# m4tx/idencomp

Measured on NVIDIA B200. Metric: fastq_compress_decompress_GBps, higher is better.
Workload: dtype u32

## Files before the change

### idencomp_b200/csrc/idn_gpu.cu

```cuda
#include "../../include/idn_gpu.h"

#include <algorithm>
#include <cstdarg>
#include <cstdio>
#include <chrono>
#include <cstring>
#include <string>
#include <vector>

#include "idn_fastq.cuh"
#include "idn_native.cuh"

using namespace idn;

namespace {

struct DevBuf {
    void* p = nullptr;
    size_t cap = 0;
    cudaError_t ensure(size_t n) {
        if (n <= cap) return cudaSuccess;
        if (p) cudaFree(p);
        p = nullptr;
        cap = 0;
// ... 248 lines not shown
#endif
    for (int i = 0; i < kNumStaticPairs; i++) {
        bool same = true;
        for (int k = 0; k < 5; k++)
            same = same && ctx->slots[acid_slot].spec_tuple[k] == kStaticPairs[i][k] && ctx->slots[q_slot].spec_tuple[k] == kStaticPairs[i][5 + k];
        if (same) return i;
    }
    return -1;
}

extern "C" int32_t idn_gpu_kernel_variant(const idn_gpu_ctx* ctx, idn_model_t acid_model, idn_model_t q_model) {
    if (!ctx) return -1;
    for (idn_model_t h : {acid_model, q_model})
        if (h < 0 || (size_t)h >= ctx->slots.size() || !ctx->slots[h].used) return -1;
    if (ctx->slots[acid_model].dev.type != IDN_MODEL_ACID || ctx->slots[q_model].dev.type != IDN_MODEL_QSCORE) return -1;
    return static_pair_index(ctx, acid_model, q_model);
}
extern "C" int32_t idn_gpu_kernel_variant_count(void) { return kNumStaticPairs; }

static unsigned debug_smem() {
    static const unsigned v = [] { const char* e = getenv("IDN_DEBUG_SMEM"); return e ? (unsigned)atoi(e) : 0u; }();
    return v;
}
#define IDN_LAUNCH_UNIFORM(idx, KERNEL, grid, st, ...)                                         \
    switch (idx) {                                                                             \
        case 0: KERNEL<true, SP0><<<grid, 128, debug_smem(), st>>>(__VA_ARGS__); break;                   \
        case 1: KERNEL<true, SP1><<<grid, 128, debug_smem(), st>>>(__VA_ARGS__); break;                   \
        case 2: KERNEL<true, SP2><<<grid, 128, debug_smem(), st>>>(__VA_ARGS__); break;                   \
        case 3: KERNEL<true, SP3><<<grid, 128, debug_smem(), st>>>(__VA_ARGS__); break;                   \
        case 4: KERNEL<true, SP4><<<grid, 128, debug_smem(), st>>>(__VA_ARGS__); break;                   \
        case 5: KERNEL<true, SP5><<<grid, 128, debug_smem(), st>>>(__VA_ARGS__); break;                   \
        case 6: KERNEL<true, SP6><<<grid, 128, debug_smem(), st>>>(__VA_ARGS__); break;                   \
        case 7: KERNEL<true, SP7><<<grid, 128, debug_smem(), st>>>(__VA_ARGS__); break;                   \
        default: KERNEL<true, DynSpecs><<<grid, 128, debug_smem(), st>>>(__VA_ARGS__); break;             \
    }

#define IDN_LAUNCH_LIST(idx, KERNEL, grid, st, ...)                                            \
    switch (idx) {                                                                             \
        case 0: KERNEL<SP0><<<grid, 128, debug_smem(), st>>>(__VA_ARGS__); break;                         \
        case 1: KERNEL<SP1><<<grid, 128, debug_smem(), st>>>(__VA_ARGS__); break;                         \
        case 2: KERNEL<SP2><<<grid, 128, debug_smem(), st>>>(__VA_ARGS__); break;                         \
        case 3: KERNEL<SP3><<<grid, 128, debug_smem(), st>>>(__VA_ARGS__); break;                         \
        case 4: KERNEL<SP4><<<grid, 128, debug_smem(), st>>>(__VA_ARGS__); break;                         \
        case 5: KERNEL<SP5><<<grid, 128, debug_smem(), st>>>(__VA_ARGS__); break;                         \
        case 6: KERNEL<SP6><<<grid, 128, debug_smem(), st>>>(__VA_ARGS__); break;                         \
        case 7: KERNEL<SP7><<<grid, 128, debug_smem(), st>>>(__VA_ARGS__); break;                         \
        default: KERNEL<DynSpecs><<<grid, 128, debug_smem(), st>>>(__VA_ARGS__); break;                   \
    }

extern "C" int32_t idn_gpu_abi_version(void) { return IDN_GPU_ABI_VERSION; }

extern "C" int32_t idn_gpu_device_count(void) {
    int n = 0;
    if (cudaGetDeviceCount(&n) != cudaSuccess) {
        (void)cudaGetLastError();
        return 0;
    }
    return n;
}

static void make_crc_tables(uint32_t* tab, uint32_t* xpow) {
    for (uint32_t i = 0; i < 256; i++) {
        uint32_t c = i;
        for (int k = 0; k < 8; k++) c = (c >> 1) ^ ((c & 1) ? 0xEDB88320u : 0);
        tab[i] = c;
    }
    auto mul = [](uint32_t a, uint32_t b) {
        uint32_t p = 0;
        for (int i = 0; i < 32; i++) {
            if (b & 0x80000000u) p ^= a;
            a = (a >> 1) ^ ((a & 1) ? 0xEDB88320u : 0);
            b <<= 1;
        }
        return p;
    };
    xpow[0] = 0x00800000u;
    for (int k = 1; k < 64; k++) xpow[k] = mul(xpow[k - 1], xpow[k - 1]);
}

static void make_crc_back_tables(const uint32_t* tab, const uint32_t* xpow, uint32_t* back ) {
    uint32_t rtop[256];
    for (uint32_t i = 0; i < 256; i++) rtop[tab[i] >> 24] = i;
    uint32_t* tinv = back;
    uint32_t* u = back + 256;
    for (uint32_t t = 0; t < 256; t++) tinv[t] = (tab[rtop[t]] << 8) | rtop[t];
    auto linv = [&](uint32_t v) { return (v << 8) ^ tinv[v >> 24]; };
    for (uint32_t b = 0; b < 256; b++) u[b] = linv(tab[b]);
    auto mul = [](uint32_t a, uint32_t b) {
        uint32_t p = 0;
        for (int i = 0; i < 32; i++) {
            if (b & 0x80000000u) p ^= a;
            a = (a >> 1) ^ ((a & 1) ? 0xEDB88320u : 0);
            b <<= 1;
        }
        return p;
    };
    uint32_t* xlen = back + 512;
    uint32_t x = 0x80000000u;
    for (uint32_t n = 0; n < kCrcLenTab; n++) {
        xlen[2 * n] = x;
        xlen[2 * n + 1] = mul(x, x);
        x = mul(x, xpow[0]);
    }
}

extern "C" int32_t idn_gpu_create(int32_t device, idn_gpu_ctx** out) {
    if (!out) return IDN_E_INVALID_ARG;
    *out = nullptr;
    int n = idn_gpu_device_count();
    if (n <= 0 || device < 0 || device >= n) return IDN_E_CUDA;
    idn_gpu_ctx* ctx = new idn_gpu_ctx();
    ctx->device = device;
    if (const char* pb = getenv("IDN_PIPE_BLOCKS")) {
        ctx->pipe_blocks = std::max(1, atoi(pb));
        ctx->pipe_blocks_set = true;
    }
    if (getenv("IDN_NO_BUCKETS")) ctx->bucket_pairs = false;
    if (const char* w = getenv("IDN_WALK")) ctx->walk_mode = strcmp(w, "serial") == 0 ? 1 : (strcmp(w, "fast") == 0 ? 2 : 0);
    auto bail = [&](const char* what) {
        fprintf(stderr, "idn_gpu_create: %s failed: %s\n", what, cudaGetErrorString(cudaGetLastError()));
        delete ctx;
        return (int32_t)IDN_E_CUDA;
    };
    if (cudaSetDevice(device) != cudaSuccess) return bail("cudaSetDevice");
    if (cudaDeviceGetAttribute(&ctx->sm_count, cudaDevAttrMultiProcessorCount, device) != cudaSuccess) return bail("cudaDeviceGetAttribute");
    if (cudaStreamCreateWithFlags(&ctx->stream, cudaStreamNonBlocking) != cudaSuccess) return bail("cudaStreamCreate");
    if (cudaEventCreateWithFlags(&ctx->ev, cudaEventDisableTiming | cudaEventBlockingSync) != cudaSuccess) return bail("cudaEventCreate");
    if (cudaMalloc(&ctx->d_models, sizeof(ModelDev) * kMaxSlots) != cudaSuccess) return bail("cudaMalloc");
    if (cudaMemset(ctx->d_models, 0, sizeof(ModelDev) * kMaxSlots) != cudaSuccess) return bail("cudaMemset");
    uint32_t tab[256], xpow[64];
    make_crc_tables(tab, xpow);
    if (cudaMalloc(&ctx->d_crc_tab, sizeof tab) != cudaSuccess) return bail("cudaMalloc");
    if (cudaMalloc(&ctx->d_xpow, sizeof xpow) != cudaSuccess) return bail("cudaMalloc");
    if (cudaMemcpy(ctx->d_crc_tab, tab, sizeof tab, cudaMemcpyHostToDevice) != cudaSuccess) return bail("cudaMemcpy");
    if (cudaMemcpy(ctx->d_xpow, xpow, sizeof xpow, cudaMemcpyHostToDevice) != cudaSuccess) return bail("cudaMemcpy");
    {
        std::vector<uint32_t> back(512 + 2 * kCrcLenTab);
        make_crc_back_tables(tab, xpow, back.data());
        if (cudaMalloc(&ctx->d_crc_back, back.size() * 4) != cudaSuccess) return bail("cudaMalloc");
        if (cudaMemcpy(ctx->d_crc_back, back.data(), back.size() * 4, cudaMemcpyHostToDevice) != cudaSuccess) return bail("cudaMemcpy");
    }
    if (getenv("IDN_NO_ENC_CRC")) ctx->enc_crc = false;
    *out = ctx;
    return IDN_OK;
}

static void pipe_destroy(idn_gpu_pipe* p);

extern "C" void idn_gpu_destroy(idn_gpu_ctx* ctx) {
    if (!ctx) return;
    cudaSetDevice(ctx->device);
    cudaDeviceSynchronize();
    for (auto& s : ctx->slots)
        if (s.used) s.free_all();
    DevBuf* bufs[] = {&ctx->w_scratch, &ctx->w_paylen,  &ctx->w_sizes,   &ctx->w_chosen,     &ctx->w_tiles,  &ctx->w_sliceoff,
                      &ctx->w_readblock, &ctx->w_small, &ctx->w_crcpart, &ctx->w_crclen,     &ctx->w_index,  &ctx->w_blk,
                      &ctx->w_lanefirst, &ctx->w_laneoff, &ctx->w_laneblock, &ctx->w_blkinfo, &ctx->w_nhdr, &ctx->w_lanesym, &ctx->w_walkdone, &ctx->w_blockadj,
                      &ctx->f_text, &ctx->f_tilecnt, &ctx->f_tilebase, &ctx->f_linestart, &ctx->f_linefn, &ctx->f_linestate, &ctx->f_tilefn,
                      &ctx->f_tilestate, &ctx->f_recscan, &ctx->f_title, &ctx->f_namelo, &ctx->f_namelen, &ctx->f_readlen, &ctx->f_readoff,
                      &ctx->f_nameoff, &ctx->f_names, &ctx->f_acids, &ctx->f_quals, &ctx->f_err, &ctx->f_fmtoff, &ctx->f_fmttext,
                      &ctx->f_blockfirst, &ctx->f_nxt, &ctx->w_bucket, &ctx->w_list,
                      &ctx->s_acids,   &ctx->s_quals,   &ctx->s_readoff, &ctx->s_blockfirst, &ctx->s_prefix, &ctx->s_names,
                      &ctx->s_nameoff, &ctx->s_out,     &ctx->s_blockoff, &ctx->s_crc,       &ctx->s_stats,  &ctx->s_sizes,
                      &ctx->s_blocks,  &ctx->s_blocklen, &ctx->s_aout,    &ctx->s_qout,    &ctx->s_offout,     &ctx->s_status, &ctx->s_idx};
    for (DevBuf* b : bufs) b->release();
    pipe_destroy(ctx->pipe);
    cudaFree(ctx->d_models);
    cudaFree(ctx->d_crc_tab);
    cudaFree(ctx->d_xpow);
    cudaFree(ctx->d_crc_back);
    if (ctx->ev) cudaEventDestroy(ctx->ev);
    if (ctx->stream) cudaStreamDestroy(ctx->stream);
    delete ctx;
}

extern "C" int32_t idn_gpu_host_alloc(uint64_t bytes, void** p) {
    if (!p) return IDN_E_INVALID_ARG;
    *p = nullptr;
    if (cudaHostAlloc(p, bytes ? bytes : 1, cudaHostAllocPortable) != cudaSuccess) {
        (void)cudaGetLastError();
        *p = nullptr;
        return IDN_E_CUDA;
    }
    return IDN_OK;
}
extern "C" void idn_gpu_host_free(void* p) {
    if (p) cudaFreeHost(p);
}

extern "C" int32_t idn_gpu_set_walk(idn_gpu_ctx* ctx, int32_t mode) {
    if (!ctx) return IDN_E_INVALID_ARG;
    if (mode < 0 || mode > 2) return fail(ctx, IDN_E_INVALID_ARG, "walk mode %d", mode);
    ctx->walk_mode = mode;
    return IDN_OK;
}

extern "C" int32_t idn_gpu_set_lane_symbols(idn_gpu_ctx* ctx, uint32_t lane_syms) {
    if (!ctx) return IDN_E_INVALID_ARG;
    if (lane_syms == 0) return fail(ctx, IDN_E_INVALID_ARG, "lane_syms must be positive");
    ctx->lane_syms = lane_syms;
    return IDN_OK;
}

extern "C" const char* idn_gpu_last_error(const idn_gpu_ctx* ctx) { return ctx ? ctx->err.c_str() : "no context"; }
extern "C" uint64_t idn_gpu_launch_count(const idn_gpu_ctx* ctx) { return ctx ? ctx->launches : 0; }

extern "C" int32_t idn_gpu_model_upload(idn_gpu_ctx* ctx, int32_t model_type, int32_t spec_kind, int32_t acid_order,
                                        int32_t q_order, int32_t pos_bits, int32_t q_max, uint32_t n_ctx,
                                        const uint16_t* cum, const uint32_t* spec_keys, const uint32_t* spec_ctx,
                                        uint64_t n_specs, idn_model_t* handle) {
    if (!ctx || !handle || !cum) return fail(ctx, IDN_E_INVALID_ARG, "NULL argument");
    if (model_type != IDN_MODEL_ACID && model_type != IDN_MODEL_QSCORE)
        return fail(ctx, IDN_E_INVALID_ARG, "bad model type %d", model_type);
    if (n_ctx > 65536) return fail(ctx, IDN_E_UNSUPPORTED, "model has %u contexts (limit 65536, check_model sequence_compressor.rs:209-219)", n_ctx);
    if (n_specs && (!spec_keys || !spec_ctx)) return fail(ctx, IDN_E_INVALID_ARG, "NULL spec table");
    CU(cudaSetDevice(ctx->device));
    const SpecBuild sb = make_spec(spec_kind, acid_order, q_order, pos_bits, q_max);
    const SpecDev spec = sb.spec;
    const uint32_t bits = sb.total_bits;
    if (!sb.ok)
// ... 1738 lines not shown
```

### idencomp_b200/csrc/idn_kernels.cuh

```cuda
#pragma once
#include "idn_device.cuh"

namespace idn {

struct BackReader {
    const uint32_t* wp;
    uint32_t word;
    int lane;
    __device__ __forceinline__ void start(const uint8_t* last) {
        const uintptr_t a = reinterpret_cast<uintptr_t>(last);
        wp = reinterpret_cast<const uint32_t*>(a & ~(uintptr_t)3);
        lane = (int)(a & 3) + 4;
        word = 0;
    }
    __device__ __forceinline__ uint32_t get() {
        if (lane >= 4) {
            word = __ldg(wp);
            lane -= 4;
        }
        const uint32_t b = (word >> (8 * lane)) & 0xffu;
        if (--lane < 0) {
            lane = 7;
            wp--;
        }
// ... 7 lines not shown
    int lane;
    __device__ __forceinline__ void start(const uint8_t* first) {
        const uintptr_t a = reinterpret_cast<uintptr_t>(first);
        wp = reinterpret_cast<const uint32_t*>(a & ~(uintptr_t)3);
        lane = (int)(a & 3) - 4;
        word = 0;
    }
    __device__ __forceinline__ uint32_t get() {
        if (lane < 0) {
            word = __ldg(wp);
            lane += 4;
        }
        const uint32_t b = (word >> (8 * lane)) & 0xffu;
        if (++lane == 4) {
            lane = -4;
            wp++;
        }
        return b;
    }
};

__device__ __forceinline__ uint4 load_chunk16(const uint8_t* __restrict__ base, unsigned long long n, const uint8_t* c) {
    if (c >= base && c + 16 <= base + n) return __ldg(reinterpret_cast<const uint4*>(c));
    uint32_t w[4] = {0, 0, 0, 0};
#pragma unroll
    for (int j = 0; j < 16; j++)
        if (c + j >= base && c + j < base + n) w[j >> 2] |= (uint32_t)__ldg(c + j) << (8 * (j & 3));
    return make_uint4(w[0], w[1], w[2], w[3]);
}

struct SymBackReader {
    const uint8_t *abase, *qbase;
    unsigned long long n;
    const uint8_t* c;
    uint32_t ca, cq;
    uint32_t a0, a1, a2, q0, q1, q2;
    uint32_t left;
    bool vec;
    __device__ __forceinline__ void load() {
        const uint4 va = load_chunk16(abase, n, c), vq = load_chunk16(qbase, n, qbase + (c - abase));
        ca = va.w; a2 = va.z; a1 = va.y; a0 = va.x;
        cq = vq.w; q2 = vq.z; q1 = vq.y; q0 = vq.x;
        c -= 16;
        left = 16;
    }
    __device__ __forceinline__ void next_word() {
        ca = a2; a2 = a1; a1 = a0;
        cq = q2; q2 = q1; q1 = q0;
    }
    __device__ __forceinline__ void start(const uint8_t* acids, const uint8_t* quals, unsigned long long n_symbols, long long off,
                                          uint32_t len) {
        abase = acids;
        qbase = quals;
        n = n_symbols;
        vec = ((reinterpret_cast<uintptr_t>(acids) ^ reinterpret_cast<uintptr_t>(quals)) & 15) == 0;
        ca = cq = a0 = a1 = a2 = q0 = q1 = q2 = 0;
        left = 0;
        const uint8_t* last = acids + off + (long long)len - 1;
        c = last;
        if (!vec || len == 0) return;
        const uint32_t k = (uint32_t)(reinterpret_cast<uintptr_t>(last) & 15);
        c = last - k;
        load();
        for (uint32_t t = 3; t > (k >> 2); t--) next_word();
        const uint32_t sh = 8 * (3 - (k & 3));
        ca <<= sh;
        cq <<= sh;
        left = k + 1;
    }
    __device__ __forceinline__ void get(uint32_t& a, uint32_t& q) {
        if (!vec) {
            a = __ldg(c);
            q = __ldg(qbase + (c - abase));
            c--;
            return;
        }
        if (left == 0) load();
        a = ca >> 24;
        q = cq >> 24;
        ca <<= 8;
        cq <<= 8;
        left--;
        if ((left & 3) == 0 && left != 0) next_word();
    }
};

struct BackWriter {
    uint32_t* wptr;
    unsigned long long acc;
    uint32_t nbits;
    __device__ __forceinline__ void init(uint8_t* end) {
        wptr = reinterpret_cast<uint32_t*>(end);
        acc = 0;
        nbits = 0;
    }
    __device__ __forceinline__ uint32_t bytes(const uint8_t* end) const {
        return (uint32_t)(reinterpret_cast<const uint32_t*>(end) - wptr) * 4u + (nbits >> 3);
    }
    __device__ __forceinline__ void push_bits(uint32_t bytes_be, uint32_t kbits) {
        acc = (acc << kbits) | bytes_be;
        nbits += kbits;
    }
    __device__ __forceinline__ void drain() {
        if (nbits >= 32) {
            nbits -= 32;
            *--wptr = (uint32_t)(acc >> nbits);
        }
    }
    __device__ __forceinline__ void push_u32_le(uint32_t x) {
        acc = (acc << 32) | x;
        nbits += 32;
        drain();
    }
    __device__ __forceinline__ void finish() {
        uint8_t* p = reinterpret_cast<uint8_t*>(wptr);
        const uint32_t n = nbits >> 3;
        for (uint32_t k = 0; k < n; k++) p[-1 - (int)k] = (uint8_t)(acc >> (8 * (n - 1 - k)));
    }
};

struct FwdWriter {
    uint8_t* wbase;
    uint32_t acc, lane, first;
    __device__ __forceinline__ void init(uint8_t* dst) {
        lane = (uint32_t)(reinterpret_cast<uintptr_t>(dst) & 3);
        first = lane;
        wbase = dst - lane;
        acc = 0;
    }
    __device__ __forceinline__ void push(uint32_t b) {
        acc |= b << (8 * lane);
        if (++lane == 4) {
            if (first == 0) {
                *reinterpret_cast<uint32_t*>(wbase) = acc;
            } else {
                for (uint32_t k = first; k < 4; k++) wbase[k] = (uint8_t)(acc >> (8 * k));
                first = 0;
            }
            wbase += 4;
            acc = 0;
            lane = 0;
        }
    }
    __device__ __forceinline__ void finish() {
        for (uint32_t k = first; k < lane; k++) wbase[k] = (uint8_t)(acc >> (8 * k));
    }
};

template <int M>
struct ModelPack {
    ModelDev m[M];
    uint32_t n;
};

template <int M, bool kDense>
__global__ void __launch_bounds__(128)
score_multi_kernel(const ModelPack<M> P, const uint8_t* __restrict__ acids, const uint8_t* __restrict__ quals,
                   const uint64_t* __restrict__ read_off, uint64_t n_reads, uint32_t n_cols, uint32_t col0,
                   uint32_t* __restrict__ sizes, uint32_t* __restrict__ err) {
    uint64_t r = (uint64_t)blockIdx.x * blockDim.x + threadIdx.x;
    if (r >= n_reads) return;
    uint64_t off = read_off[r];
    uint32_t len = (uint32_t)(read_off[r + 1] - off);
    uint32_t pbmax = 0;
#pragma unroll
    for (int k = 0; k < M; k++)
// ... 89 lines not shown
        uint32_t res[kMaxCand + 1];
        for (uint32_t s = 0; s <= n_cand; s++) res[s] = pick_model(sz, n_cand, s == n_cand ? NONE : s);
        for (uint32_t s = 0; s <= n_cand; s++) {
            uint32_t cur = out[s];
            out[s] = res[cur == NONE ? n_cand : cur];
        }
    }
    uint32_t in_state = NONE;
    for (uint32_t l = 0; l < 31; l++) {
        uint32_t my_out = out[in_state == NONE ? n_cand : in_state];
        uint32_t from_l = __shfl_sync(0xffffffffu, my_out, l);
        if (lane == l + 1) in_state = from_l;
    }
    uint32_t cur = in_state;
    for (uint64_t r = c0; r < c1; r++) {
        for (uint32_t k = 0; k < n_cand; k++) sz[k] = sizes ? sizes[r * n_models + cols[k]] : 0u;
        uint32_t best = pick_model(sz, n_cand, cur);
        ch[r] = (uint8_t)best;
        sw[r] = best != cur;
        cur = best;
    }
}

__global__ void switch_single_kernel(const uint32_t* __restrict__ block_first, uint32_t n_blocks, uint8_t* __restrict__ switched,
                                     uint64_t n_reads) {
    uint32_t b = blockIdx.x * blockDim.x + threadIdx.x;
    if (b >= n_blocks || block_first[b + 1] == block_first[b]) return;
    switched[block_first[b]] = 1;
    switched[n_reads + block_first[b]] = 1;
}

struct EncodeArgs {
    const ModelDev* models;
    const uint8_t* acids;
    const uint8_t* quals;
    uint64_t n_symbols;
    const uint64_t* read_off;
    uint64_t n_reads;
    int32_t fixed_acid, fixed_q;
    const uint8_t* chosen;
    const int32_t* cand_model;
    uint8_t* scratch;
    uint32_t* pay_len;
    uint32_t* err;
    const uint8_t* switched;
    const uint8_t* cand_index;
    const uint32_t* crc_back;
    const uint32_t* xpow;
    uint32_t* part_crc;
    unsigned long long* part_len;
};
struct ReadList {
    const uint32_t* list;
    const uint32_t* base;
    const uint32_t* count;
};
constexpr unsigned long long kSlotExtra = 24;

struct EncStream {
    uint32_t x0, x1;
    BackWriter out;
    bool bad;
    __device__ __forceinline__ void begin(uint8_t* slot_end) {
        x0 = x1 = kRansL;
        out.init(slot_end);
        bad = false;
    }
    __device__ __forceinline__ void flush_states() {
        out.push_u32_le(x0);
        out.push_u32_le(x1);
    }
    __device__ __forceinline__ void flush() {
        flush_states();
        out.finish();
    }
    __device__ __forceinline__ uint32_t total(const uint8_t* slot_end) const { return out.bytes(slot_end); }
};

constexpr uint32_t kCrcLenTab = 1024;
__device__ __forceinline__ uint32_t gf2_mul(uint32_t a, uint32_t b);
__device__ __forceinline__ uint32_t x8n_mod_p(unsigned long long n, const uint32_t* __restrict__ xpow);
struct EncCrc {
    const uint32_t* tinv;
    const uint32_t* u;
    uint32_t ba, bq;
    __device__ __forceinline__ void add(uint32_t a, uint32_t q) {
        ba = (ba << 8) ^ tinv[ba >> 24] ^ u[a];
        bq = (bq << 8) ^ tinv[bq >> 24] ^ u[q];
    }
};

template <class P>
__device__ __forceinline__ void encode_read_body(const ModelDev& ma, const ModelDev& mq, const uint8_t* __restrict__ acids,
                                                 const uint8_t* __restrict__ quals, unsigned long long n_symbols, long long off,
                                                 uint32_t len, uint32_t p0, uint32_t p1, EncStream& S, EncCrc& C) {
    constexpr SpecDev ksa = P::sa(), ksq = P::sq();
    const SpecDev& sa = P::kStatic ? ksa : ma.spec;
    const SpecDev& sq = P::kStatic ? ksq : mq.spec;
#ifndef IDN_NO_SYM16
    SymBackReader rs;
    rs.start(acids, quals, n_symbols, off, p1);
#else
    (void)n_symbols;
    BackReader ra, rq;
    ra.start(acids + off + p1 - 1);
    rq.start(quals + off + p1 - 1);
#endif
    GenBack ga, gq;
    ga.clear(sa);
    gq.clear(sq);
    int32_t front = (int32_t)p1 - 1;
    uint32_t raw_a = 0;
    unsigned long long raw_q = 0;
    auto pull = [&]() {
        uint32_t a = 0, q = 0;
        if (front >= 0) {
#ifndef IDN_NO_SYM16
            rs.get(a, q);
#else
            a = ra.get();
            q = rq.get();
#endif
            if (a > 4 || q > 93) {
                S.bad = true;
                a = a > 4 ? 0 : a;
                q = q > 93 ? 0 : q;
            }
            if (C.tinv) C.add(a, q);
        }
        front--;
        const bool z = a * q == 0;
        ga.shift_in(sa, a, q, z);
        gq.shift_in(sq, a, q, z);
        raw_a = (raw_a >> 3) | (a << (3 * kHist));
        raw_q = (raw_q >> 7) | ((unsigned long long)q << (7 * kHist));
    };
#pragma unroll 1
    for (int t = 0; t < kHist; t++) pull();
    ga.init_state(sa);
    gq.init_state(sq);
    const uint32_t pbmax = sa.pb > sq.pb ? sa.pb : sq.pb;
    const uint32_t psa = pbmax - sa.pb, psq = pbmax - sq.pb;
    PosBack pb;
    pb.init_at(len, pbmax, p1);

#ifndef IDN_NO_AENC
    const bool direct_a = P::kStatic || ma.aenc != nullptr;
#else
    const bool direct_a = false;
#endif
    const uint2* __restrict__ enc_a = direct_a ? ma.aenc : ma.enc;
    int32_t j = (int32_t)p1;
    auto rows_next = [&](uint32_t& row_a, uint32_t& row_q) {
        j--;
        row_a = row_q = 0;
        if (j >= (int32_t)p0) {
            pull();
            ga.step_back(sa);
            gq.step_back(sq);
            pb.retreat();
            row_a = direct_a ? ga.index(sa, pb.pos, psa) : gen_row<P::kStatic>(ma, sa, ga, pb.pos, psa);
            row_q = gen_row<P::kStatic>(mq, sq, gq, pb.pos, psq);
        }
    };
    uint32_t row_a, row_q;
    rows_next(row_a, row_q);
    uint2 ea = make_uint2(0, 0), eq = make_uint2(0, 0);
    if (p1 > p0) {
        ea = ldg_stream8(enc_a + (row_a * kAcidSyms + (raw_a & 7u)));
        eq = __ldg(mq.enc + (row_q * kQSyms + ((uint32_t)raw_q & 127u)));
    }
    rows_next(row_a, row_q);
#pragma unroll 1
    for (uint32_t i = p1; i-- > p0;) {
        uint2 ea_n = make_uint2(0, 0), eq_n = make_uint2(0, 0);
        if (i > p0) {
            ea_n = ldg_stream8(enc_a + (row_a * kAcidSyms + (raw_a & 7u)));
            eq_n = __ldg(mq.enc + (row_q * kQSyms + ((uint32_t)raw_q & 127u)));
        }
        rows_next(row_a, row_q);
        rans_put_bf(S.x0, ea, S.out);
        rans_put_bf(S.x1, eq, S.out);
        S.out.drain();
        ea = ea_n;
        eq = eq_n;
    }
}

#ifndef IDN_ENC_MINB
#define IDN_ENC_MINB 8
#endif
#ifndef IDN_DEC_MINB
#define IDN_DEC_MINB 8
#endif
template <bool kUniform, class P>
__device__ __forceinline__ void encode_one(const EncodeArgs& A, const ModelDev& MA, const ModelDev& MQ, uint64_t r, const uint32_t* s_back) {
    int32_t ia = A.fixed_acid, iq = A.fixed_q;
    if (!kUniform && A.chosen) {
        ia = A.cand_model[A.chosen[r]];
        iq = A.cand_model[kMaxCand + A.chosen[A.n_reads + r]];
    }
    const ModelDev& ma = kUniform ? MA : A.models[ia];
    const ModelDev& mq = kUniform ? MQ : A.models[iq];
    const long long off = (long long)A.read_off[r];
    const uint32_t len = (uint32_t)(A.read_off[r + 1] - A.read_off[r]);
    EncStream S;
    S.begin(A.scratch + 4ull * A.read_off[r + 1] + kSlotExtra * (r + 1));
    EncCrc C{A.crc_back ? s_back : nullptr, s_back + 256, 0u, 0u};
    encode_read_body<P>(ma, mq, A.acids, A.quals, A.n_symbols, off, len, 0, len, S, C);
    if (A.crc_back) {
        uint32_t x1, x2;
        if (len < kCrcLenTab) {
            const uint2 x = __ldg(reinterpret_cast<const uint2*>(A.crc_back + 512) + len);
            x1 = x.x;
            x2 = x.y;
        } else {
            x1 = x8n_mod_p(len, A.xpow);
            x2 = gf2_mul(x1, x1);
        }
        A.part_crc[r] = len ? ~(gf2_mul(x1, C.bq) ^ gf2_mul(x2, ~C.ba)) : 0u;
        A.part_len[r] = 2ull * len;
    }
    S.flush_states();
    const uint32_t plen = S.total(A.scratch + 4ull * A.read_off[r + 1] + kSlotExtra * (r + 1));
    A.pay_len[r] = plen;
    S.out.push_u32_le(__byte_perm(len, 0, 0x0123));
    S.out.push_u32_le(__byte_perm(plen, 0, 0x0123));
    S.out.push_bits(2u, 8);
    S.out.drain();
    if (A.switched) {
        if (A.switched[A.n_reads + r]) {
            S.out.push_bits(((uint32_t)A.cand_index[kMaxCand + A.chosen[A.n_reads + r]] << 8) | 1u, 16);
            S.out.drain();
        }
        if (A.switched[r]) {
            S.out.push_bits(((uint32_t)A.cand_index[A.chosen[r]] << 8) | 1u, 16);
            S.out.drain();
        }
    }
    S.out.finish();
    if (S.bad) atomicOr(A.err, 1u);
}

template <bool kUniform, class P>
__global__ void __launch_bounds__(128, kUniform ? IDN_ENC_MINB : 1)
encode_kernel(EncodeArgs A, const ModelDev MA, const ModelDev MQ) {
    __shared__ uint32_t s_back[512];
    if (A.crc_back) {
        for (int i = threadIdx.x; i < 512; i += blockDim.x) s_back[i] = A.crc_back[i];
        __syncthreads();
    }
    uint64_t r = (uint64_t)blockIdx.x * blockDim.x + threadIdx.x;
    if (r >= A.n_reads) return;
    encode_one<kUniform, P>(A, MA, MQ, r, s_back);
}

template <class P>
__global__ void __launch_bounds__(128, IDN_ENC_MINB)
encode_list_kernel(EncodeArgs A, const ModelDev MA, const ModelDev MQ, ReadList L) {
    __shared__ uint32_t s_back[512];
    if (A.crc_back) {
        for (int i = threadIdx.x; i < 512; i += blockDim.x) s_back[i] = A.crc_back[i];
        __syncthreads();
    }
    const uint32_t n = *L.count;
    const uint32_t* __restrict__ list = L.list + *L.base;
    for (uint64_t i = (uint64_t)blockIdx.x * blockDim.x + threadIdx.x; i < n; i += (uint64_t)gridDim.x * blockDim.x)
        encode_one<true, P>(A, MA, MQ, list[i], s_back);
}

constexpr uint32_t kMaxPairs = 1024;

struct EncodePairKey {
    const uint8_t* chosen;
    uint64_t n_reads;
    uint32_t n_q;
    __device__ __forceinline__ uint32_t operator()(uint64_t r) const {
        return r < n_reads ? (uint32_t)chosen[r] * n_q + chosen[n_reads + r] : 0xffffffffu;
    }
};

template <class KeyFn>
__global__ void __launch_bounds__(256)
bucket_count_kernel(KeyFn key, uint64_t n, uint32_t n_pairs, uint32_t* __restrict__ cnt) {
    __shared__ uint32_t hist[kMaxPairs];
    for (uint32_t k = threadIdx.x; k < n_pairs; k += blockDim.x) hist[k] = 0;
    __syncthreads();
    const uint64_t r = (uint64_t)blockIdx.x * blockDim.x + threadIdx.x;
    const uint32_t k = r < n ? key(r) : 0xffffffffu;
    if (k < n_pairs) atomicAdd(&hist[k], 1u);
    __syncthreads();
    for (uint32_t j = threadIdx.x; j < n_pairs; j += blockDim.x)
        if (hist[j]) atomicAdd(&cnt[j], hist[j]);
}

__global__ void bucket_base_kernel(const uint32_t* __restrict__ cnt, uint32_t n_pairs, uint32_t* __restrict__ base, uint32_t* __restrict__ cursor) {
    if (threadIdx.x != 0 || blockIdx.x != 0) return;
    uint32_t acc = 0;
    for (uint32_t k = 0; k < n_pairs; k++) {
        base[k] = cursor[k] = acc;
        acc += cnt[k];
    }
}

template <class KeyFn>
__global__ void __launch_bounds__(256)
bucket_scatter_kernel(KeyFn key, uint64_t n, uint32_t n_pairs, uint32_t* __restrict__ cursor, uint32_t* __restrict__ list) {
    __shared__ uint32_t hist[kMaxPairs];
    for (uint32_t k = threadIdx.x; k < n_pairs; k += blockDim.x) hist[k] = 0;
    __syncthreads();
    const uint64_t r = (uint64_t)blockIdx.x * blockDim.x + threadIdx.x;
    const uint32_t k = r < n ? key(r) : 0xffffffffu;
    uint32_t rank = 0;
    if (k < n_pairs) rank = atomicAdd(&hist[k], 1u);
    __syncthreads();
    for (uint32_t j = threadIdx.x; j < n_pairs; j += blockDim.x)
        if (hist[j]) hist[j] = atomicAdd(&cursor[j], hist[j]);
    __syncthreads();
    if (k < n_pairs) list[hist[k] + rank] = (uint32_t)r;
}

constexpr int kScanBlock = 256;
constexpr int kScanItems = 8;
constexpr int kScanTile = kScanBlock * kScanItems;

__device__ __forceinline__ unsigned long long block_exclusive_scan(unsigned long long v, unsigned long long* total,
                                                                  unsigned long long* smem ) {
    uint32_t lane = threadIdx.x & 31, wid = threadIdx.x >> 5;
    unsigned long long inc = v;
    for (int d = 1; d < 32; d <<= 1) {
        unsigned long long o = __shfl_up_sync(0xffffffffu, inc, d);
        if (lane >= (uint32_t)d) inc += o;
    }
    if (lane == 31) smem[wid] = inc;
    __syncthreads();
    if (wid == 0) {
        unsigned long long s = lane < kScanBlock / 32 ? smem[lane] : 0;
        unsigned long long sinc = s;
        for (int d = 1; d < 32; d <<= 1) {
            unsigned long long o = __shfl_up_sync(0xffffffffu, sinc, d);
            if (lane >= (uint32_t)d) sinc += o;
        }
        if (lane < kScanBlock / 32) smem[lane] = sinc - s;
        if (lane == kScanBlock / 32 - 1) *total = sinc;
    }
// ... 1349 lines not shown
```

### idencomp_b200/csrc/idn_native.cuh

```cuda
#pragma once
#include "idn_kernels.cuh"

namespace idn {

constexpr uint32_t kNativeHdrFixed = 1 + 4 + 4 + 4 + 4 + 1 + 4;

__device__ __forceinline__ void store_u32be(uint8_t* p, uint32_t v) {
    p[0] = (uint8_t)(v >> 24);
    p[1] = (uint8_t)(v >> 16);
    p[2] = (uint8_t)(v >> 8);
    p[3] = (uint8_t)v;
}

constexpr uint32_t kNativeMinSplitQ = 256;
constexpr uint32_t kNativeHistBytes = 2 * kHist;

__host__ __device__ __forceinline__ uint32_t native_pieces(uint32_t len, uint32_t Q) {
    return (Q >= kNativeMinSplitQ && len > Q) ? (len + Q - 1) / Q : 1u;
}

struct LaneCount {
    const uint64_t* read_off;
    const uint32_t* block_first;
    const uint32_t* read_block;
// ... 18 lines not shown
                    uint32_t* __restrict__ lane_first, unsigned long long* __restrict__ lane_sym) {
    uint64_t r = (uint64_t)blockIdx.x * blockDim.x + threadIdx.x;
    if (r == 0) {
        lane_first[lane_scan[n_reads]] = (uint32_t)n_reads;
        lane_sym[lane_scan[n_reads]] = fn.read_off[n_reads];
    }
    if (r >= n_reads) return;
    unsigned long long l = lane_scan[r];
    const uint32_t len = (uint32_t)(fn.read_off[r + 1] - fn.read_off[r]);
    const uint32_t pc = native_pieces(len, fn.lane_syms);
    if (fn.first_piece_opens(r)) {
        lane_first[l] = (uint32_t)r;
        lane_sym[l] = fn.read_off[r];
        l++;
    }
    for (uint32_t j = 1; j < pc; j++, l++) {
        lane_first[l] = (uint32_t)r;
        lane_sym[l] = fn.read_off[r] + (unsigned long long)j * fn.lane_syms;
    }
}

__global__ void __launch_bounds__(128)
lane_choose_kernel(const uint32_t* __restrict__ sizes, uint32_t n_cols, const uint32_t* __restrict__ cand_cols,
                   const uint32_t* __restrict__ n_cand2, const uint32_t* __restrict__ has_sizes,
                   const uint32_t* __restrict__ lane_first, const unsigned long long* __restrict__ lane_sym,
                   const uint64_t* __restrict__ read_off, uint64_t n_reads, const unsigned long long* __restrict__ n_lanes_dev,
                   uint64_t lane_cap, uint8_t* __restrict__ lane_choice ) {
    uint64_t t = (uint64_t)blockIdx.x * blockDim.x + threadIdx.x;
    uint64_t l = t >> 1;
    uint32_t type = (uint32_t)t & 1;
    if (l >= *n_lanes_dev) return;
    uint32_t best = 0;
    if (has_sizes[type]) {
        const unsigned long long a = lane_sym[l], b = lane_sym[l + 1];
        unsigned long long best_sum = ~0ull;
        for (uint32_t k = 0; k < n_cand2[type]; k++) {
            uint32_t col = cand_cols[type * kMaxCand + k];
            unsigned long long sum = 0;
            for (uint64_t r = lane_first[l]; r < n_reads && read_off[r] < b; r++)
                if (read_off[r + 1] > a) sum += sizes[r * n_cols + col];
            if (sum < best_sum) {
                best_sum = sum;
                best = k;
            }
        }
    }
    lane_choice[(size_t)type * lane_cap + l] = (uint8_t)best;
}

struct EncodeLaneArgs {
    const ModelDev* models;
    const uint8_t* acids;
    const uint8_t* quals;
    uint64_t n_symbols;
    const uint64_t* read_off;
    uint64_t n_reads;
    const uint32_t* lane_first;
    const unsigned long long* lane_sym;
    const unsigned long long* n_lanes_dev;
    uint64_t lane_cap;
    const uint8_t* lane_choice;
    const int32_t* cand_model;
    uint8_t* scratch;
    uint32_t* lane_len;
    uint32_t* err;
};
constexpr unsigned long long kLaneSlotExtra = 8 + kNativeHistBytes;

#ifndef IDN_LANE_MINB
#define IDN_LANE_MINB 8
#endif
template <bool kUniform, class P>
__device__ __forceinline__ void encode_lane_one(const EncodeLaneArgs& A, const ModelDev& MA, const ModelDev& MQ, uint64_t l64) {
    const uint32_t l = (uint32_t)l64;
    const uint32_t r_lo = A.lane_first[l];
    int32_t ia = 0, iq = 0;
    if (!kUniform) {
        ia = A.cand_model[A.lane_choice ? A.lane_choice[l] : 0];
        iq = A.cand_model[kMaxCand + (A.lane_choice ? A.lane_choice[A.lane_cap + l] : 0)];
    }
    const ModelDev& ma = kUniform ? MA : A.models[ia];
    const ModelDev& mq = kUniform ? MQ : A.models[iq];
    EncStream S;
    EncCrc C{nullptr, nullptr, 0u, 0u};
    S.begin(A.scratch + 4ull * A.lane_sym[l + 1] + kLaneSlotExtra * ((unsigned long long)l + 1));
    if (A.lane_sym[l + 1] > A.lane_sym[l]) {
        uint32_t r = A.lane_first[l + 1] < A.n_reads ? A.lane_first[l + 1] : (uint32_t)A.n_reads - 1;
        while (r > r_lo && A.read_off[r] >= A.lane_sym[l + 1]) r--;
#pragma unroll 1
        for (;; r--) {
            const unsigned long long a = A.lane_sym[l], b = A.lane_sym[l + 1];
            const unsigned long long ro = A.read_off[r], re = A.read_off[r + 1];
            if (re > a && ro < b) {
                const uint32_t p0 = (uint32_t)((a > ro ? a : ro) - ro), p1 = (uint32_t)((b < re ? b : re) - ro);
                encode_read_body<P>(ma, mq, A.acids, A.quals, A.n_symbols, (long long)ro, (uint32_t)(re - ro), p0, p1, S, C);
            }
            if (r == r_lo) break;
        }
    }
    S.flush_states();
    {
        const unsigned long long a = A.lane_sym[l], b = A.lane_sym[l + 1];
        if (b > a && a > A.read_off[r_lo]) {
            const uint8_t* ha = A.acids + a - kHist;
            const uint8_t* hq = A.quals + a - kHist;
            auto word = [](const uint8_t* p) { return (uint32_t)p[0] | ((uint32_t)p[1] << 8) | ((uint32_t)p[2] << 16) | ((uint32_t)p[3] << 24); };
            S.out.push_u32_le(word(hq + 4));
            S.out.push_u32_le(word(hq));
            S.out.push_u32_le(word(ha + 4));
            S.out.push_u32_le(word(ha));
        }
    }
    S.out.finish();
    A.lane_len[l] = S.total(A.scratch + 4ull * A.lane_sym[l + 1] + kLaneSlotExtra * ((unsigned long long)l + 1));
    if (S.bad) atomicOr(A.err, 1u);
}

template <bool kUniform, class P>
__global__ void __launch_bounds__(128, kUniform ? IDN_LANE_MINB : 1)
encode_lane_kernel(EncodeLaneArgs A, const ModelDev MA, const ModelDev MQ) {
    const uint64_t l64 = (uint64_t)blockIdx.x * blockDim.x + threadIdx.x;
    if (l64 >= *A.n_lanes_dev) return;
    encode_lane_one<kUniform, P>(A, MA, MQ, l64);
}

template <class P>
__global__ void __launch_bounds__(128, IDN_LANE_MINB)
encode_lane_list_kernel(EncodeLaneArgs A, const ModelDev MA, const ModelDev MQ, ReadList L) {
    const uint32_t n = *L.count;
    const uint32_t* __restrict__ list = L.list + *L.base;
    for (uint64_t i = (uint64_t)blockIdx.x * blockDim.x + threadIdx.x; i < n; i += (uint64_t)gridDim.x * blockDim.x)
        encode_lane_one<true, P>(A, MA, MQ, list[i]);
}

struct EncodeLanePairKey {
    const uint8_t* lane_choice;
    const unsigned long long* n_lanes_dev;
    uint64_t lane_cap;
    uint32_t n_q;
    __device__ __forceinline__ uint32_t operator()(uint64_t l) const {
        return l < *n_lanes_dev ? (uint32_t)lane_choice[l] * n_q + lane_choice[lane_cap + l] : 0xffffffffu;
    }
};

struct LaneLenFn {
    const uint32_t* lane_len;
    const unsigned long long* n_lanes_dev;
    __device__ __forceinline__ unsigned long long operator()(uint64_t l) const { return l < *n_lanes_dev ? lane_len[l] : 0; }
};

__global__ void __launch_bounds__(256)
native_block_info_kernel(const uint64_t* __restrict__ read_off, const uint32_t* __restrict__ block_first, uint32_t n_blocks,
                         const unsigned long long* __restrict__ lane_scan , uint32_t lane_syms,
                         uint32_t* __restrict__ blk_width ,
                         uint32_t* __restrict__ blk_const_len, uint32_t* __restrict__ blk_lane0 ) {
    __shared__ uint32_t s_min[256], s_max[256];
    uint32_t b = blockIdx.x;
    if (b >= n_blocks) return;
    uint64_t r0 = block_first[b], r1 = block_first[b + 1];
    uint32_t mn = 0xffffffffu, mx = 0;
    for (uint64_t r = r0 + threadIdx.x; r < r1; r += blockDim.x) {
        uint32_t len = (uint32_t)(read_off[r + 1] - read_off[r]);
        mn = min(mn, len);
        mx = max(mx, len);
    }
    s_min[threadIdx.x] = mn;
    s_max[threadIdx.x] = mx;
// ... 493 lines not shown
```

Before: 269.0.

## Process encoder symbols a word at a time and simplify backward CRC update

Adds a word-at-a-time fast path to the per-read rANS encode loop. It peeks four acid and quality bytes at once, validates them with a packed SWAR range check, and feeds them through the history and entropy coder in an unrolled loop. The backward CRC drops the u[] lookup table, XORs raw bytes directly, and gains a word-level update, so the CRC back table and its shared-memory copy shrink to 256 entries. This is meant to cut per-symbol branching, byte loads and table lookups, at the cost of more complex alignment and bound logic (wlim/skip) and a CRC formula change whose correctness depends on the reworked table algebra.

```diff
diff --git a/idencomp_b200/csrc/idn_gpu.cu b/idencomp_b200/csrc/idn_gpu.cu
--- a/idencomp_b200/csrc/idn_gpu.cu
+++ b/idencomp_b200/csrc/idn_gpu.cu
@@ -354,10 +354,7 @@
     uint32_t rtop[256];
     for (uint32_t i = 0; i < 256; i++) rtop[tab[i] >> 24] = i;
     uint32_t* tinv = back;
-    uint32_t* u = back + 256;
     for (uint32_t t = 0; t < 256; t++) tinv[t] = (tab[rtop[t]] << 8) | rtop[t];
-    auto linv = [&](uint32_t v) { return (v << 8) ^ tinv[v >> 24]; };
-    for (uint32_t b = 0; b < 256; b++) u[b] = linv(tab[b]);
     auto mul = [](uint32_t a, uint32_t b) {
         uint32_t p = 0;
         for (int i = 0; i < 32; i++) {
@@ -367,7 +364,7 @@
         }
         return p;
     };
-    uint32_t* xlen = back + 512;
+    uint32_t* xlen = back + 256;
     uint32_t x = 0x80000000u;
     for (uint32_t n = 0; n < kCrcLenTab; n++) {
         xlen[2 * n] = x;
@@ -407,7 +404,7 @@
     if (cudaMemcpy(ctx->d_crc_tab, tab, sizeof tab, cudaMemcpyHostToDevice) != cudaSuccess) return bail("cudaMemcpy");
     if (cudaMemcpy(ctx->d_xpow, xpow, sizeof xpow, cudaMemcpyHostToDevice) != cudaSuccess) return bail("cudaMemcpy");
     {
-        std::vector<uint32_t> back(512 + 2 * kCrcLenTab);
+        std::vector<uint32_t> back(256 + 2 * kCrcLenTab);
         make_crc_back_tables(tab, xpow, back.data());
         if (cudaMalloc(&ctx->d_crc_back, back.size() * 4) != cudaSuccess) return bail("cudaMalloc");
         if (cudaMemcpy(ctx->d_crc_back, back.data(), back.size() * 4, cudaMemcpyHostToDevice) != cudaSuccess) return bail("cudaMemcpy");
diff --git a/idencomp_b200/csrc/idn_kernels.cuh b/idencomp_b200/csrc/idn_kernels.cuh
--- a/idencomp_b200/csrc/idn_kernels.cuh
+++ b/idencomp_b200/csrc/idn_kernels.cuh
@@ -113,6 +113,19 @@
         cq <<= 8;
         left--;
         if ((left & 3) == 0 && left != 0) next_word();
+    }
+    __device__ __forceinline__ void peek_word() {
+        if (left == 0) {
+            const uint4 va = __ldg(reinterpret_cast<const uint4*>(c)), vq = __ldg(reinterpret_cast<const uint4*>(qbase + (c - abase)));
+            ca = va.w; a2 = va.z; a1 = va.y; a0 = va.x;
+            cq = vq.w; q2 = vq.z; q1 = vq.y; q0 = vq.x;
+            c -= 16;
+            left = 16;
+        }
+    }
+    __device__ __forceinline__ void skip_word() {
+        left -= 4;
+        next_word();
     }
 };
 
@@ -368,11 +381,19 @@
 __device__ __forceinline__ uint32_t x8n_mod_p(unsigned long long n, const uint32_t* __restrict__ xpow);
 struct EncCrc {
     const uint32_t* tinv;
-    const uint32_t* u;
     uint32_t ba, bq;
     __device__ __forceinline__ void add(uint32_t a, uint32_t q) {
-        ba = (ba << 8) ^ tinv[ba >> 24] ^ u[a];
-        bq = (bq << 8) ^ tinv[bq >> 24] ^ u[q];
+        ba = (ba << 8) ^ tinv[ba >> 24] ^ a;
+        bq = (bq << 8) ^ tinv[bq >> 24] ^ q;
+    }
+    __device__ __forceinline__ void add_word(uint32_t wa, uint32_t wq) {
+#pragma unroll
+        for (int k = 0; k < 4; k++) {
+            ba = (ba << 8) ^ tinv[ba >> 24];
+            bq = (bq << 8) ^ tinv[bq >> 24];
+        }
+        ba ^= wa;
+        bq ^= wq;
     }
 };
 
@@ -395,10 +416,16 @@
     GenBack ga, gq;
     ga.clear(sa);
     gq.clear(sq);
-    int32_t front = (int32_t)p1 - 1;
     uint32_t raw_a = 0;
     unsigned long long raw_q = 0;
-    auto pull = [&]() {
+    auto shift_in = [&](uint32_t a, uint32_t q) {
+        const bool z = a * q == 0;
+        ga.shift_in(sa, a, q, z);
+        gq.shift_in(sq, a, q, z);
+        raw_a = (raw_a >> 3) | (a << (3 * kHist));
+        raw_q = (raw_q >> 7) | ((unsigned long long)q << (7 * kHist));
+    };
+    auto pull = [&](int32_t front) {
         uint32_t a = 0, q = 0;
         if (front >= 0) {
 #ifndef IDN_NO_SYM16
@@ -414,15 +441,10 @@
             }
             if (C.tinv) C.add(a, q);
         }
-        front--;
-        const bool z = a * q == 0;
-        ga.shift_in(sa, a, q, z);
-        gq.shift_in(sq, a, q, z);
-        raw_a = (raw_a >> 3) | (a << (3 * kHist));
-        raw_q = (raw_q >> 7) | ((unsigned long long)q << (7 * kHist));
+        shift_in(a, q);
     };
 #pragma unroll 1
-    for (int t = 0; t < kHist; t++) pull();
+    for (int t = 0; t < kHist; t++) pull((int32_t)p1 - 1 - t);
     ga.init_state(sa);
     gq.init_state(sq);
     const uint32_t pbmax = sa.pb > sq.pb ? sa.pb : sq.pb;
@@ -436,38 +458,79 @@
     const bool direct_a = false;
 #endif
     const uint2* __restrict__ enc_a = direct_a ? ma.aenc : ma.enc;
-    int32_t j = (int32_t)p1;
-    auto rows_next = [&](uint32_t& row_a, uint32_t& row_q) {
-        j--;
+    uint32_t row_a, row_q;
+    auto gen_step = [&]() {
+        ga.step_back(sa);
+        gq.step_back(sq);
+        pb.retreat();
+        row_a = direct_a ? ga.index(sa, pb.pos, psa) : gen_row<P::kStatic>(ma, sa, ga, pb.pos, psa);
+        row_q = gen_row<P::kStatic>(mq, sq, gq, pb.pos, psq);
+    };
+    auto rows_next = [&](int32_t j) {
         row_a = row_q = 0;
         if (j >= (int32_t)p0) {
-            pull();
-            ga.step_back(sa);
-            gq.step_back(sq);
-            pb.retreat();
-            row_a = direct_a ? ga.index(sa, pb.pos, psa) : gen_row<P::kStatic>(ma, sa, ga, pb.pos, psa);
-            row_q = gen_row<P::kStatic>(mq, sq, gq, pb.pos, psq);
+            pull(j - kHist);
+            gen_step();
         }
     };
-    uint32_t row_a, row_q;
-    rows_next(row_a, row_q);
+    auto entries = [&](uint2& ea_, uint2& eq_) {
+        ea_ = ldg_stream8(enc_a + (row_a * kAcidSyms + (raw_a & 7u)));
+        eq_ = __ldg(mq.enc + (row_q * kQSyms + ((uint32_t)raw_q & 127u)));
+    };
     uint2 ea = make_uint2(0, 0), eq = make_uint2(0, 0);
-    if (p1 > p0) {
-        ea = ldg_stream8(enc_a + (row_a * kAcidSyms + (raw_a & 7u)));
-        eq = __ldg(mq.enc + (row_q * kQSyms + ((uint32_t)raw_q & 127u)));
-    }
-    rows_next(row_a, row_q);
-#pragma unroll 1
-    for (uint32_t i = p1; i-- > p0;) {
-        uint2 ea_n = make_uint2(0, 0), eq_n = make_uint2(0, 0);
-        if (i > p0) {
-            ea_n = ldg_stream8(enc_a + (row_a * kAcidSyms + (raw_a & 7u)));
-            eq_n = __ldg(mq.enc + (row_q * kQSyms + ((uint32_t)raw_q & 127u)));
-        }
-        rows_next(row_a, row_q);
+    auto put = [&]() {
         rans_put_bf(S.x0, ea, S.out);
         rans_put_bf(S.x1, eq, S.out);
         S.out.drain();
+    };
+    rows_next((int32_t)p1 - 1);
+    if (p1 > p0) entries(ea, eq);
+    rows_next((int32_t)p1 - 2);
+#ifndef IDN_NO_SYM16
+    const long long skip = (long long)((0 - reinterpret_cast<uintptr_t>(acids)) & 15) - off;
+    uint32_t wlim = p0 > kHist ? p0 : kHist;
+    if (skip > 0 && (uint32_t)skip + kHist > wlim) wlim = (uint32_t)skip + kHist;
+    wlim += 4 + 2;
+#endif
+    uint32_t i = p1;
+#pragma unroll 1
+    while (i > p0) {
+#ifndef IDN_NO_SYM16
+        if (rs.vec && (rs.left & 3) == 0 && i >= wlim) {
+            rs.peek_word();
+            if ((((rs.ca & 0x7f7f7f7fu) + 0x7b7b7b7bu) | rs.ca | ((rs.cq & 0x7f7f7f7fu) + 0x22222222u) | rs.cq) & 0x80808080u) {
+                S.bad = true;
+                uint32_t ca = 0, cq = 0;
+#pragma unroll 1
+                for (int k = 0; k < 32; k += 8) {
+                    const uint32_t a = (rs.ca >> k) & 0xffu, q = (rs.cq >> k) & 0xffu;
+                    ca |= (a > 4 ? 0u : a) << k;
+                    cq |= (q > 93 ? 0u : q) << k;
+                }
+                rs.ca = ca;
+                rs.cq = cq;
+            }
+            if (C.tinv) C.add_word(rs.ca, rs.cq);
+#pragma unroll
+            for (int k = 0; k < 4; k++) {
+                uint2 ea_n, eq_n;
+                entries(ea_n, eq_n);
+                shift_in(__byte_perm(rs.ca, 0, 0x4443 - k), __byte_perm(rs.cq, 0, 0x4443 - k));
+                gen_step();
+                put();
+                ea = ea_n;
+                eq = eq_n;
+            }
+            rs.skip_word();
+            i -= 4;
+            continue;
+        }
+#endif
+        i--;
+        uint2 ea_n = make_uint2(0, 0), eq_n = make_uint2(0, 0);
+        if (i > p0) entries(ea_n, eq_n);
+        rows_next((int32_t)i - 2);
+        put();
         ea = ea_n;
         eq = eq_n;
     }
@@ -492,12 +555,12 @@
     const uint32_t len = (uint32_t)(A.read_off[r + 1] - A.read_off[r]);
     EncStream S;
     S.begin(A.scratch + 4ull * A.read_off[r + 1] + kSlotExtra * (r + 1));
-    EncCrc C{A.crc_back ? s_back : nullptr, s_back + 256, 0u, 0u};
+    EncCrc C{A.crc_back ? s_back : nullptr, 0u, 0u};
     encode_read_body<P>(ma, mq, A.acids, A.quals, A.n_symbols, off, len, 0, len, S, C);
     if (A.crc_back) {
         uint32_t x1, x2;
         if (len < kCrcLenTab) {
-            const uint2 x = __ldg(reinterpret_cast<const uint2*>(A.crc_back + 512) + len);
+            const uint2 x = __ldg(reinterpret_cast<const uint2*>(A.crc_back + 256) + len);
             x1 = x.x;
             x2 = x.y;
         } else {
@@ -531,9 +594,9 @@
 template <bool kUniform, class P>
 __global__ void __launch_bounds__(128, kUniform ? IDN_ENC_MINB : 1)
 encode_kernel(EncodeArgs A, const ModelDev MA, const ModelDev MQ) {
-    __shared__ uint32_t s_back[512];
+    __shared__ uint32_t s_back[256];
     if (A.crc_back) {
-        for (int i = threadIdx.x; i < 512; i += blockDim.x) s_back[i] = A.crc_back[i];
+        for (int i = threadIdx.x; i < 256; i += blockDim.x) s_back[i] = A.crc_back[i];
         __syncthreads();
     }
     uint64_t r = (uint64_t)blockIdx.x * blockDim.x + threadIdx.x;
@@ -544,9 +607,9 @@
 template <class P>
 __global__ void __launch_bounds__(128, IDN_ENC_MINB)
 encode_list_kernel(EncodeArgs A, const ModelDev MA, const ModelDev MQ, ReadList L) {
-    __shared__ uint32_t s_back[512];
+    __shared__ uint32_t s_back[256];
     if (A.crc_back) {
-        for (int i = threadIdx.x; i < 512; i += blockDim.x) s_back[i] = A.crc_back[i];
+        for (int i = threadIdx.x; i < 256; i += blockDim.x) s_back[i] = A.crc_back[i];
         __syncthreads();
     }
     const uint32_t n = *L.count;
diff --git a/idencomp_b200/csrc/idn_native.cuh b/idencomp_b200/csrc/idn_native.cuh
--- a/idencomp_b200/csrc/idn_native.cuh
+++ b/idencomp_b200/csrc/idn_native.cuh
@@ -124,7 +124,7 @@
     const ModelDev& ma = kUniform ? MA : A.models[ia];
     const ModelDev& mq = kUniform ? MQ : A.models[iq];
     EncStream S;
-    EncCrc C{nullptr, nullptr, 0u, 0u};
+    EncCrc C{nullptr, 0u, 0u};
     S.begin(A.scratch + 4ull * A.lane_sym[l + 1] + kLaneSlotExtra * ((unsigned long long)l + 1));
     if (A.lane_sym[l + 1] > A.lane_sym[l]) {
         uint32_t r = A.lane_first[l + 1] < A.n_reads ? A.lane_first[l + 1] : (uint32_t)A.n_reads - 1;
```

New measurement: 283.9, median of 6. +5.5%, better.
